# JuliaGaussianProcesses/AbstractGPs.jl

Measured on NVIDIA H100. Metric: ms to logpdf(fx,y)+posterior(fx,y), lower is better.
Workload: dtype f64

## Files before the change

abstractgps.jl_b200/csrc/engine.cu:

```cuda
#include <cuda_runtime.h>
#include <math.h>
#include <stdio.h>
#include <stdlib.h>
#include <string.h>
#include <functional>
#include <string>
#include <type_traits>
#include <utility>
#include <vector>

#include <nccl.h>

#include "agp.h"
#include "kernels.h"
#include "umma_ozaki.h"

#define TILE AGP_TILE

struct agp_ctx {
  int device = 0;
  cudaStream_t stream = nullptr;
  cudaStream_t stream2 = nullptr;
  cudaStream_t stream3 = nullptr;
  cudaEvent_t ev_s3 = nullptr, ev_fac = nullptr;
  bool s3_dirty = false;
  std::vector<cudaEvent_t> dep_ev;
  agp_config cfg{};
  std::string err;
  int64_t info = 0;
  int memspace = AGP_MEM_HOST;
  bool out_dev_override = false;
  double timings[8] = {0, 0, 0, 0, 0, 0, 0, 0};
  cudaEvent_t ev[8]{};
  std::vector<cudaEvent_t> prof_ev;
  int prof_used = 0;
  int profile = 1;
  int rank = 0, nranks = 1, grid_p = 1, grid_q = 1;
  ncclComm_t nccl = nullptr;
  OzakiWs oz{};
  OzakiWs oz2{};
  int64_t oz_rows = 0, oz2_rows = 0;
  cudaStream_t stream_comm = nullptr;
  int oz_S = 6;
  int oz_chunk = 16;
  int oz_S32 = 4;
};

struct CompState {
  CompositeDesc desc{};
  std::vector<double> w;
  int64_t grad_len = 5;
  bool owns_w = false;
};

struct agp_post {
  agp_ctx* ctx = nullptr;
  int dtype = AGP_F64;
  int64_t n = 0, n_pad = 0, lda = 0;
  int D = 0;
  void* L = nullptr;
  void* Dinv = nullptr;
  void* Xt = nullptr;
  void* alpha = nullptr;
  void* ard = nullptr;
  void* delta = nullptr;
  unsigned char* valid = nullptr;
  std::vector<std::pair<int64_t, int64_t>> segs;
  agp_kernel k{};
  int mean_kind = 0;
  double mean_c = 0.0;
  double logdet = 0.0;
  int dist_R = 0, dist_me = 0, dist_G = 0, dist_nloc = 0;
  int64_t dist_W = 0;
  void* Lloc = nullptr;
  void* Dinv_loc = nullptr;
  CompState* comp = nullptr;
};

struct agp_vfe_post {
  agp_ctx* ctx = nullptr;
  int dtype = AGP_F32;
  int64_t m = 0, m_pad = 0, lda = 0;
  int D = 0;
  void* U = nullptr;
  void* Udinv = nullptr;
  void* Lam = nullptr;
  void* Ldinv = nullptr;
  void* Zt = nullptr;
  void* m_e = nullptr;
  void* ard = nullptr;
  agp_kernel k{};
  int mean_kind = 0;
  double mean_c = 0.0;
};

namespace {

static inline int64_t round_up(int64_t x, int64_t m) { return (x + m - 1) / m * m; }
static inline int64_t env_int64(const char* name, int64_t dflt) {
  const char* v = getenv(name);
  return v ? atoll(v) : dflt;
}

#define CK(call)                                                                          \
  do {                                                                                    \
    cudaError_t _e = (call);                                                              \
    if (_e != cudaSuccess) {                                                              \
      char _b[512];                                                                       \
      snprintf(_b, sizeof(_b), "%s:%d %s -> %s", __FILE__, __LINE__, #call, cudaGetErrorString(_e)); \
      ctx->err = _b;                                                                      \
      return AGP_ERR_CUDA;                                                                \
    }                                                                                     \
  } while (0)

#define CKN(call)                                                                         \
  do {                                                                                    \
    ncclResult_t _r = (call);                                                             \
    if (_r != ncclSuccess) {                                                              \
      char _b[512];                                                                       \
      snprintf(_b, sizeof(_b), "%s:%d %s -> %s", __FILE__, __LINE__, #call, ncclGetErrorString(_r)); \
      ctx->err = _b;                                                                      \
      return AGP_ERR_NCCL;                                                                \
    }                                                                                     \
  } while (0)

template <typename T> struct NcclType;
template <> struct NcclType<float> { static constexpr ncclDataType_t v = ncclFloat; };
template <> struct NcclType<double> { static constexpr ncclDataType_t v = ncclDouble; };

struct Scratch {
  agp_ctx* ctx;
  std::vector<void*> ptrs;
  explicit Scratch(agp_ctx* c) : ctx(c) {}
  ~Scratch() { for (void* p : ptrs) cudaFreeAsync(p, ctx->stream); }
  cudaError_t alloc(void** p, size_t bytes) {
    if (bytes == 0) bytes = 16;
    cudaError_t e = cudaMallocAsync(p, bytes, ctx->stream);
    if (e == cudaSuccess) ptrs.push_back(*p);
    return e;
  }
  void release(void* p) {
    for (auto& q : ptrs) if (q == p) { q = ptrs.back(); ptrs.pop_back(); return; }
  }
};

template <typename T>
int upload(agp_ctx* ctx, Scratch& sc, const void* src, size_t count, bool always_host, T** out) {
  if (!src || count == 0) { *out = nullptr; return AGP_OK; }
  if (!always_host && ctx->memspace == AGP_MEM_DEVICE) { *out = (T*)src; return AGP_OK; }
  void* d = nullptr;
  CK(sc.alloc(&d, count * sizeof(T)));
  CK(cudaMemcpyAsync(d, src, count * sizeof(T), cudaMemcpyHostToDevice, ctx->stream));
  *out = (T*)d;
  return AGP_OK;
}

template <typename T>
int download(agp_ctx* ctx, void* dst, const T* src, size_t count, bool always_host) {
  if (!dst || count == 0) return AGP_OK;
  cudaMemcpyKind kind = (!always_host && (ctx->memspace == AGP_MEM_DEVICE || ctx->out_dev_override)) ? cudaMemcpyDeviceToDevice : cudaMemcpyDeviceToHost;
  CK(cudaMemcpyAsync(dst, src, count * sizeof(T), kind, ctx->stream));
  return AGP_OK;
}

int check_kernel(agp_ctx* ctx, const agp_kernel* k, int D) {
  if (!k) { ctx->err = "kernel spec is NULL"; return AGP_ERR_INVALID; }
  if (k->family == AGP_COMPOSITE) {
    if (ctx->nccl) { ctx->err = "composite kernels are supported on a single-GPU context only"; return AGP_ERR_UNSUPPORTED; }
    if (k->transform != AGP_T_NONE || k->variance != 1.0) {
      ctx->err = "a composite kernel takes transform AGP_T_NONE and variance 1 (scalings belong to the terms)";
      return AGP_ERR_INVALID;
    }
    if (D <= 0) { ctx->err = "D must be positive"; return AGP_ERR_DIM_MISMATCH; }
    return AGP_OK;
  }
  if (k->family < AGP_SE || k->family > AGP_LINEAR) { ctx->err = "unsupported kernel family"; return AGP_ERR_UNSUPPORTED; }
  if (k->transform < AGP_T_NONE || k->transform > AGP_T_ARD) { ctx->err = "unsupported transform"; return AGP_ERR_UNSUPPORTED; }
  if (k->transform == AGP_T_ARD && !k->ard) { ctx->err = "ARD transform without weights"; return AGP_ERR_INVALID; }
  if (D <= 0) { ctx->err = "D must be positive"; return AGP_ERR_DIM_MISMATCH; }
  return AGP_OK;
}

template <typename T>
int comp_build(agp_ctx* ctx, const agp_kernel* k, int D, CompState* cs) {
  const agp_kernel_composite* c = k->composite;
  if (!c || !c->nfactors || !c->variance || !c->factors) { ctx->err = "composite kernel without its descriptor"; return AGP_ERR_INVALID; }
  if (k->transform != AGP_T_NONE || k->variance != 1.0) {
    ctx->err = "a composite kernel takes transform AGP_T_NONE and variance 1 (scalings belong to the terms)";
    return AGP_ERR_INVALID;
  }
  if (c->nterms < 1 || c->nterms > AGP_COMP_MAX) { ctx->err = "composite kernel: 1..8 terms"; return AGP_ERR_INVALID; }
  int nf = 0;
  for (int t = 0; t < c->nterms; ++t) {
    if (c->nfactors[t] < 1) { ctx->err = "composite kernel: every term needs at least one factor"; return AGP_ERR_INVALID; }
    nf += c->nfactors[t];
    if (nf > AGP_COMP_MAX) { ctx->err = "composite kernel: at most 8 factors in all"; return AGP_ERR_INVALID; }
  }
  CompositeDesc& d = cs->desc;
  d = CompositeDesc{};
  d.nterms = c->nterms;
  d.nfactors = nf;
  cs->w.clear();
  int raw_sq = -1, raw_dot = -1;
  auto new_acc = [&](int kind) {
    const int a = d.nacc++;
    d.acc_kind[a] = kind;
    cs->w.resize((size_t)2 * d.nacc * D, 0.0);
    for (int i = 0; i < D; ++i) cs->w[(size_t)2 * a * D + i] = 1.0;
    return a;
  };
  int64_t slot = 5;
  int f = 0;
  for (int t = 0; t < c->nterms; ++t) {
    d.variance[t] = c->variance[t];
    d.g_var[t] = (int)slot++;
    for (int j = 0; j < c->nfactors[t]; ++j, ++f) {
      const agp_kernel_factor& in = c->factors[f];
      CompFactor& F = d.f[f];
      F.family = in.family; F.transform = in.transform; F.term = t;
      F.s = in.transform == AGP_T_SCALE ? in.scale : 1.0;
      F.s2 = 1.0; F.param = in.param;
      F.g_s = F.g_p = F.g_w = F.g_r = -1;
      if (in.family < AGP_SE || in.family > AGP_CONSTANT) { ctx->err = "composite kernel: unsupported factor family"; return AGP_ERR_UNSUPPORTED; }
      if (in.transform < AGP_T_NONE || in.transform > AGP_T_ARD) { ctx->err = "composite kernel: unsupported factor transform"; return AGP_ERR_UNSUPPORTED; }
      if (in.transform == AGP_T_ARD && !in.ard) { ctx->err = "composite kernel: ARD factor without weights"; return AGP_ERR_INVALID; }
      if (in.family == AGP_RQ && !(in.param > 0.0)) { ctx->err = "composite kernel: RationalQuadratic alpha must be > 0"; return AGP_ERR_INVALID; }
      const T* ard = (const T*)in.ard;
      if (in.family == AGP_CONSTANT) {
        F.acc = -1;
      } else if (in.family == AGP_PERIODIC) {
        F.acc = new_acc(COMP_ACC_PER);
        for (int i = 0; i < D; ++i) {
          const double r = in.r ? (double)((const T*)in.r)[i] : 1.0;
          if (!(r > 0.0)) { ctx->err = "composite kernel: Periodic r must be > 0"; return AGP_ERR_INVALID; }
          cs->w[(size_t)2 * F.acc * D + i] = in.transform == AGP_T_ARD ? (double)ard[i] : F.s;
          cs->w[(size_t)(2 * F.acc + 1) * D + i] = 1.0 / r;
        }
      } else if (in.transform == AGP_T_ARD) {
        F.acc = new_acc(in.family == AGP_LINEAR ? COMP_ACC_DOT : COMP_ACC_SQ);
        for (int i = 0; i < D; ++i) cs->w[(size_t)2 * F.acc * D + i] = (double)ard[i];
      } else if (in.family == AGP_LINEAR) {
        if (raw_dot < 0) raw_dot = new_acc(COMP_ACC_DOT);
        F.acc = raw_dot;
        F.s2 = F.s * F.s;
      } else {
        if (raw_sq < 0) raw_sq = new_acc(COMP_ACC_SQ);
        F.acc = raw_sq;
        F.s2 = F.s * F.s;
      }
      if (in.transform == AGP_T_SCALE) F.g_s = (int)slot++;
      else if (in.transform == AGP_T_ARD) { F.g_w = (int)slot; slot += D; }
      if (in.family == AGP_RQ || in.family == AGP_LINEAR || in.family == AGP_CONSTANT) F.g_p = (int)slot++;
      if (in.family == AGP_PERIODIC) { F.g_r = (int)slot; slot += D; }
    }
  }
  if (d.nacc == 0) new_acc(COMP_ACC_SQ);
  cs->grad_len = slot;
  return AGP_OK;
}

template <typename T>
int comp_upload(agp_ctx* ctx, Scratch& sc, CompState* cs, bool own) {
  std::vector<T> h(cs->w.begin(), cs->w.end());
  void* dv = nullptr;
  const size_t bytes = h.size() * sizeof(T);
  if (own) CK(cudaMallocAsync(&dv, bytes, ctx->stream));
  else CK(sc.alloc(&dv, bytes));
  CK(cudaMemcpyAsync(dv, h.data(), bytes, cudaMemcpyHostToDevice, ctx->stream));
  CK(cudaStreamSynchronize(ctx->stream));
  cs->desc.w = dv;
  cs->owns_w = own;
  return AGP_OK;
}

void comp_free(CompState* cs, cudaStream_t s) {
  if (!cs) return;
  if (cs->owns_w && cs->desc.w) cudaFreeAsync((void*)cs->desc.w, s);
  delete cs;
}

void prof_begin(agp_ctx* ctx) { ctx->prof_used = 0; }
cudaEvent_t prof_event(agp_ctx* ctx) {
  if (ctx->prof_used == (int)ctx->prof_ev.size()) {
    cudaEvent_t e;
    cudaEventCreate(&e);
    ctx->prof_ev.push_back(e);
  }
  return ctx->prof_ev[ctx->prof_used++];
}
double prof_total_ms(agp_ctx* ctx) {
  double t = 0;
  for (int i = 0; i + 1 < ctx->prof_used; i += 2) {
    float ms = 0;
    if (cudaEventElapsedTime(&ms, ctx->prof_ev[i], ctx->prof_ev[i + 1]) == cudaSuccess) t += ms;
  }
  return t;
}

static cudaEvent_t dep_event(agp_ctx* ctx, size_t i) {
  while (ctx->dep_ev.size() <= i) {
    cudaEvent_t e;
    cudaEventCreateWithFlags(&e, cudaEventDisableTiming);
    ctx->dep_ev.push_back(e);
  }
  return ctx->dep_ev[i];
}

template <typename T>
void trailing_update(agp_ctx* ctx, T* L, int64_t lda, int64_t row0, int64_t col0, int64_t kcol0, int64_t K,
                     int64_t M, int64_t N, cudaStream_t st, const OzakiWs* oz = nullptr, int64_t oz_row0 = 0) {
  if (M <= 0 || N <= 0) return;
  if (ctx->profile) cudaEventRecord(prof_event(ctx), st);
  bool done = false;
  if (oz) {
    if constexpr (std::is_same<T, double>::value) {
      done = ozaki_syrk(*oz, L + row0 + col0 * lda, lda, M, N, 1, 0, 0, col0 - oz_row0, row0 - oz_row0, st) == 0;
    } else {
      done = ozaki_update_ex(*oz, L + row0 + col0 * lda, 1, lda, M, N, 0, -1.0, 0, 0, col0 - oz_row0, row0 - oz_row0, st) == 0;
    }
  }
  if (!done) {
    GemmArgs u{};
    u.A = L + row0 + kcol0 * lda; u.lda = lda;
    u.B = L + row0 + kcol0 * lda; u.ldb = lda;
    u.C = L + row0 + col0 * lda; u.ldc = lda;
    u.M = M; u.N = N; u.K = K; u.alpha_neg = 1; u.beta_one = 1; u.lower_only = 1;
    if (row0 != col0) { u.b_tile_stride = TILE; u.b_off = col0 - row0; }
    launch_gemm<T>(u, st);
  }
  if (ctx->profile) cudaEventRecord(prof_event(ctx), st);
}

static void join_inverses(agp_ctx* ctx) {
  if (!ctx->s3_dirty) return;
  cudaEventRecord(ctx->ev_s3, ctx->stream3);
  cudaStreamWaitEvent(ctx->stream, ctx->ev_s3, 0);
  ctx->s3_dirty = false;
}

static int resolve_G(const agp_ctx* ctx, int64_t n_pad) {
  int nb = ctx->cfg.tile_nb;
  if (nb <= 0) nb = (n_pad >= 8192) ? 512 : TILE;
  int G = nb / TILE;
  if (G > 8) G = 8;
  return G < 1 ? 1 : G;
}
static int resolve_fp64_mode(const agp_ctx* ctx, int64_t n_pad) {
  if (ctx->cfg.fp64_mode >= 0) return ctx->cfg.fp64_mode;
  return n_pad >= 8192 ? 1 : 0;
}
static int resolve_fp32_mode(const agp_ctx* ctx, int64_t n_pad) {
  if (ctx->cfg.fp32_mode >= 0) return ctx->cfg.fp32_mode;
  return n_pad >= 4096 ? 1 : 0;
}
template <typename T> static int resolve_tensor_mode(const agp_ctx* ctx, int64_t n_pad) {
  return std::is_same<T, double>::value ? resolve_fp64_mode(ctx, n_pad) : resolve_fp32_mode(ctx, n_pad);
}
struct OzFmt { int S, bits; };
template <typename T> static OzFmt slice_format(const agp_ctx* ctx, int64_t K, bool factor) {
  if (!std::is_same<T, double>::value) return {ctx->oz_S32, 7};
  if (ctx->oz_S == 6) return (factor && K <= OZ8_MAX_K) ? OzFmt{6, 8} : OzFmt{7, 7};
  return {ctx->oz_S, 7};
}
static bool ensure_ws(OzakiWs& ws, int64_t& ws_rows, int64_t rows, int K, OzFmt f, cudaStream_t s) {
  if (!ws.SL || ws.K != K || ws_rows < rows || ws.S != f.S || ws.bits != f.bits) {
    if (ws.SL) ozaki_ws_destroy(&ws, s);
    if (ozaki_ws_create(&ws, rows, K, f.S, s, f.bits) == 0) ws_rows = rows;
    else { memset(&ws, 0, sizeof(ws)); ws_rows = 0; }
  }
  return ws.SL != nullptr;
}
template <typename T> static bool ensure_oz2(agp_ctx* ctx, int64_t rows, int K, bool factor, cudaStream_t s) {
  return ensure_ws(ctx->oz2, ctx->oz2_rows, rows, K, slice_format<T>(ctx, K, factor), s);
}
template <typename T> static bool ensure_oz(agp_ctx* ctx, int64_t rows, int K, bool factor, cudaStream_t s) {
  return ensure_ws(ctx->oz, ctx->oz_rows, rows, K, slice_format<T>(ctx, K, factor), s);
}

template <typename T>
int panel_route(int64_t rows_below) {
  if (!std::is_same<T, double>::value || !potrf_split_enabled()) return AGP_PANEL_FUSED;
  static const int64_t trsm_gemm_min = env_int64("AGP_TRSM_GEMM_MIN", 8192);
  return rows_below >= trsm_gemm_min ? AGP_PANEL_SPLIT_GEMM : AGP_PANEL_SPLIT_SUBST;
}

template <typename T>
void panel_block(agp_ctx* ctx, int route, T* Akk, int64_t lda, int64_t rows_below, T* Dinv_k, double* logdet_part,
                 int blk, int* info, cudaStream_t s) {
  if constexpr (std::is_same<T, double>::value) {
    if (route == AGP_PANEL_SPLIT_SUBST) {
      launch_potrf_factor_f64(Akk, lda, logdet_part, blk, info, s);
      cudaEventRecord(ctx->ev_fac, s);
      cudaStreamWaitEvent(ctx->stream3, ctx->ev_fac, 0);
      launch_trtri_f64(Akk, lda, Dinv_k, ctx->stream3);
      ctx->s3_dirty = true;
      if (rows_below > 0) launch_trsm_sub_f64(Akk + TILE, lda, rows_below, Akk, s);
      return;
    }
    if (route == AGP_PANEL_SPLIT_GEMM) {
      launch_potrf_factor_f64(Akk, lda, logdet_part, blk, info, s);
      launch_trtri_f64(Akk, lda, Dinv_k, s);
    }
  }
  if (route == AGP_PANEL_FUSED) launch_potrf_diag<T>(Akk, lda, Dinv_k, logdet_part, blk, info, s);
  if (rows_below > 0) {
    GemmArgs t{};
    t.A = Akk + TILE; t.lda = lda; t.B = Dinv_k; t.ldb = TILE;
    t.C = Akk + TILE; t.ldc = lda; t.M = rows_below; t.N = TILE; t.K = TILE;
    launch_gemm<T>(t, s);
  }
}

template <typename T>
void factor_panel_step(agp_ctx* ctx, T* Lp, int64_t lda, int Gp, int g, int64_t rows, T* Dinv_p, double* logdet_part,
                       int blk_base, int* info, cudaStream_t s) {
  T* Akk = Lp + (int64_t)g * TILE + (int64_t)g * TILE * lda;
  const int64_t rows_below = rows - (int64_t)(g + 1) * TILE;
  panel_block<T>(ctx, panel_route<T>(rows_below), Akk, lda, rows_below, Dinv_p + (int64_t)g * TILE * TILE, logdet_part,
                 blk_base + g, info, s);
  if (rows_below <= 0) return;
  const int64_t ncols_in = (int64_t)(Gp - (g + 1)) * TILE;
  if (ncols_in > 0) {
    GemmArgs u{};
    u.A = Akk + TILE; u.lda = lda; u.B = Akk + TILE; u.ldb = lda;
    u.C = Akk + TILE + (int64_t)TILE * lda; u.ldc = lda;
    u.M = rows_below; u.N = ncols_in; u.K = TILE; u.alpha_neg = 1; u.beta_one = 1; u.lower_only = 1;
    launch_gemm<T>(u, s);
  }
}

template <typename T>
void factor_panel(agp_ctx* ctx, T* Lp, int64_t lda, int Gp, int64_t rows, T* Dinv_p, double* logdet_part, int blk_base,
                  int* info, cudaStream_t s) {
  for (int g = 0; g < Gp; ++g) factor_panel_step<T>(ctx, Lp, lda, Gp, g, rows, Dinv_p, logdet_part, blk_base, info, s);
}

template <typename T>
void cholesky_inplace(agp_ctx* ctx, T* L, int64_t lda, int64_t n_pad, int64_t rows_total, T* Dinv,
                      double* logdet_part, int* info) {
  cudaStream_t s = ctx->stream, s2 = ctx->stream2;
  const int nblk = (int)(n_pad / TILE);
  const int fp64_mode = resolve_tensor_mode<T>(ctx, n_pad);
  int G = resolve_G(ctx, n_pad);
  if (!std::is_same<T, double>::value && fp64_mode == 1 && ctx->cfg.tile_nb <= 0 && n_pad >= 4096) G = 4;
  const bool oz_ok = fp64_mode == 1 && nblk > 2 * G && ensure_oz<T>(ctx, rows_total, G * TILE, true, s) &&
                     (std::is_same<T, double>::value || ctx->oz.bulk == 2);
  const bool la = ctx->cfg.lookahead != 0 && nblk > 2 * G;
  const bool la2 = la && ctx->cfg.lookahead >= 2;
  bool rest_pending = false, restA_pending = false, last_rest_full = false;
  size_t ev_idx = 0, last_rest = 0, last_restA = 0;
  for (int ko = 0; ko < nblk; ko += G) {
    const int g_end = (ko + G < nblk) ? ko + G : nblk;
    factor_panel<T>(ctx, L + (int64_t)ko * TILE + (int64_t)ko * TILE * lda, lda, g_end - ko, rows_total - (int64_t)ko * TILE,
                    Dinv + (int64_t)ko * TILE * TILE, logdet_part, ko, info, s);
    const int64_t t0 = (int64_t)g_end * TILE;
    const int64_t cols_trail = n_pad - t0;
    if (cols_trail <= 0) continue;
    const int64_t K = (int64_t)(g_end - ko) * TILE, kc0 = (int64_t)ko * TILE;
    const OzakiWs* oz = nullptr;
    if (oz_ok && K == ctx->oz.K && cols_trail >= 2 * TILE) oz = &ctx->oz;
    constexpr int is_f32 = std::is_same<T, double>::value ? 0 : 1;
    if (!la) {
      if (oz) ozaki_prepare_ex(*oz, L + t0 + kc0 * lda, is_f32, 0, lda, rows_total - t0, 0, s);
      trailing_update<T>(ctx, L, lda, t0, t0, kc0, K, rows_total - t0, cols_trail, s, oz, t0);
      continue;
    }
    if (la2 && !oz) {
      cudaEvent_t e_panel = dep_event(ctx, ev_idx++), e_restA = dep_event(ctx, ev_idx++), e_restB = dep_event(ctx, ev_idx++);
      if (restA_pending) cudaStreamWaitEvent(s, dep_event(ctx, last_restA), 0);
      if (rest_pending && last_rest_full) cudaStreamWaitEvent(s, dep_event(ctx, last_rest), 0);
      cudaEventRecord(e_panel, s);
      const int64_t next_cols = (cols_trail < (int64_t)G * TILE) ? cols_trail : (int64_t)G * TILE;
      trailing_update<T>(ctx, L, lda, t0, t0, kc0, K, rows_total - t0, next_cols, s, nullptr, t0);
      restA_pending = false;
      rest_pending = false;
      if (cols_trail > next_cols) {
        const int64_t r0 = t0 + next_cols;
        const int64_t colsA = (n_pad - r0 < (int64_t)G * TILE) ? (n_pad - r0) : (int64_t)G * TILE;
        cudaStreamWaitEvent(s2, e_panel, 0);
        trailing_update<T>(ctx, L, lda, r0, r0, kc0, K, rows_total - r0, colsA, s2, nullptr, t0);
        cudaEventRecord(e_restA, s2);
        restA_pending = true;
        last_restA = ev_idx - 2;
        const int64_t r1 = r0 + colsA;
        if (n_pad > r1) trailing_update<T>(ctx, L, lda, r1, r1, kc0, K, rows_total - r1, n_pad - r1, s2, nullptr, t0);
        cudaEventRecord(e_restB, s2);
        rest_pending = true;
        last_rest_full = false;
        last_rest = ev_idx - 1;
      }
      continue;
    }
    cudaEvent_t e_panel = dep_event(ctx, ev_idx++), e_rest = dep_event(ctx, ev_idx++);
    if (rest_pending) cudaStreamWaitEvent(s, dep_event(ctx, last_rest), 0);
    if (restA_pending) { cudaStreamWaitEvent(s, dep_event(ctx, last_restA), 0); restA_pending = false; }
    if (oz) ozaki_prepare_ex(*oz, L + t0 + kc0 * lda, is_f32, 0, lda, rows_total - t0, 0, s);
    cudaEventRecord(e_panel, s);
    const int64_t next_cols = (cols_trail < (int64_t)G * TILE) ? cols_trail : (int64_t)G * TILE;
    trailing_update<T>(ctx, L, lda, t0, t0, kc0, K, rows_total - t0, next_cols, s, oz, t0);
    rest_pending = false;
    if (cols_trail > next_cols) {
      const int64_t r0 = t0 + next_cols;
      cudaStreamWaitEvent(s2, e_panel, 0);
      if (oz) oz->chunk_tiles = ctx->oz_chunk;
      trailing_update<T>(ctx, L, lda, r0, r0, kc0, K, rows_total - r0, n_pad - r0, s2, oz, t0);
      if (oz) oz->chunk_tiles = 0;
      cudaEventRecord(e_rest, s2);
      rest_pending = true;
      last_rest_full = true;
      last_rest = ev_idx - 1;
    }
  }
  if (rest_pending) cudaStreamWaitEvent(s, dep_event(ctx, last_rest), 0);
  join_inverses(ctx);
}

template <typename T>
bool forward_subst_multi_tc(agp_ctx* ctx, const T* L, int64_t lda, const T* Dinv, int64_t n_pad, T* B, int64_t ldb,
                            int64_t ncols) {
  cudaStream_t s = ctx->stream;
  constexpr int GW = 4;
  const int64_t W = (int64_t)GW * TILE;
  const int nblk = (int)(n_pad / TILE);
  constexpr int is_f32 = std::is_same<T, double>::value ? 0 : 1;
  const int64_t a_rows = round_up(n_pad, TILE);
  if (!ensure_oz<T>(ctx, a_rows + ncols, (int)W, false, s) || ctx->oz.bulk != 2) return false;
  const OzakiWs& ws = ctx->oz;
  for (int ko = 0; ko < nblk; ko += GW) {
    const int k_end = (ko + GW < nblk) ? ko + GW : nblk;
    const int64_t blk_end = (int64_t)k_end * TILE;
    for (int k = ko; k < k_end; ++k) {
      T* Bk = B + (int64_t)k * TILE;
      GemmArgs a{};
      a.A = Dinv + (int64_t)k * TILE * TILE; a.lda = TILE; a.a_kmajor = 0;
      a.B = Bk; a.ldb = ldb; a.b_kmajor = 1;
      a.C = Bk; a.ldc = ldb; a.M = TILE; a.N = ncols; a.K = TILE;
      launch_gemm<T>(a, s);
      const int64_t rows_in = blk_end - (int64_t)(k + 1) * TILE;
      if (rows_in <= 0) continue;
      GemmArgs u{};
      u.A = L + (int64_t)(k + 1) * TILE + (int64_t)k * TILE * lda; u.lda = lda; u.a_kmajor = 0;
      u.B = Bk; u.ldb = ldb; u.b_kmajor = 1;
      u.C = Bk + TILE; u.ldc = ldb; u.M = rows_in; u.N = ncols; u.K = TILE; u.alpha_neg = 1; u.beta_one = 1;
      launch_gemm<T>(u, s);
    }
    const int64_t rows_below = n_pad - blk_end, Kw = blk_end - (int64_t)ko * TILE;
    if (rows_below <= 0) continue;
    if (Kw != W) {
      GemmArgs u{};
      u.A = L + blk_end + (int64_t)ko * TILE * lda; u.lda = lda; u.a_kmajor = 0;
      u.B = B + (int64_t)ko * TILE; u.ldb = ldb; u.b_kmajor = 1;
      u.C = B + blk_end; u.ldc = ldb; u.M = rows_below; u.N = ncols; u.K = Kw; u.alpha_neg = 1; u.beta_one = 1;
      launch_gemm<T>(u, s);
      continue;
    }
    ozaki_prepare_ex(ws, L + blk_end + (int64_t)ko * TILE * lda, is_f32, 0, lda, rows_below, 0, s);
    ozaki_prepare_ex(ws, B + (int64_t)ko * TILE, is_f32, 1, ldb, ncols, a_rows, s);
    if (ozaki_update_ex(ws, B + blk_end, is_f32, ldb, rows_below, ncols, 1, -1.0, 0, 0, a_rows, 0, s) != 0) return false;
  }
  return true;
}

template <typename T>
void forward_subst_multi(agp_ctx* ctx, const T* L, int64_t lda, const T* Dinv, int64_t n_pad, T* B, int64_t ldb,
                         int64_t ncols) {
  cudaStream_t s = ctx->stream;
  const int nblk = (int)(n_pad / TILE);
  static const int64_t tc_min_cols = env_int64("AGP_SOLVE_TC_MIN_COLS", 512);
  if (resolve_tensor_mode<T>(ctx, n_pad >= 2048 ? (int64_t)1 << 20 : 0) == 1 && n_pad >= 2048 && ncols % TILE == 0 &&
      ncols >= tc_min_cols) {
    if (forward_subst_multi_tc<T>(ctx, L, lda, Dinv, n_pad, B, ldb, ncols)) return;
  }
  for (int k = 0; k < nblk; ++k) {
    T* Bk = B + (int64_t)k * TILE;
    GemmArgs a{};
    a.A = Dinv + (int64_t)k * TILE * TILE; a.lda = TILE; a.a_kmajor = 0;
    a.B = Bk; a.ldb = ldb; a.b_kmajor = 1;
    a.C = Bk; a.ldc = ldb; a.M = TILE; a.N = ncols; a.K = TILE;
    launch_gemm<T>(a, s);
    const int64_t rows_below = n_pad - (int64_t)(k + 1) * TILE;
    if (rows_below <= 0) continue;
    GemmArgs u{};
    u.A = L + (int64_t)(k + 1) * TILE + (int64_t)k * TILE * lda; u.lda = lda; u.a_kmajor = 0;
    u.B = Bk; u.ldb = ldb; u.b_kmajor = 1;
    u.C = Bk + TILE; u.ldc = ldb; u.M = rows_below; u.N = ncols; u.K = TILE; u.alpha_neg = 1; u.beta_one = 1;
    launch_gemm<T>(u, s);
  }
}

template <typename T>
bool backward_subst_multi_tc(agp_ctx* ctx, const T* L, int64_t lda, const T* Dinv, int64_t n_pad, T* B, int64_t ldb,
                             int64_t ncols) {
  cudaStream_t s = ctx->stream;
  constexpr int GW = 4;
  const int64_t W = (int64_t)GW * TILE;
  const int nblk = (int)(n_pad / TILE);
  constexpr int is_f32 = std::is_same<T, double>::value ? 0 : 1;
  const int64_t a_rows = round_up(n_pad, TILE);
  if (!ensure_oz<T>(ctx, a_rows + ncols, (int)W, false, s) || ctx->oz.bulk != 2) return false;
  const OzakiWs& ws = ctx->oz;
  for (int ko = (nblk - 1) / GW * GW; ko >= 0; ko -= GW) {
    const int k_end = (ko + GW < nblk) ? ko + GW : nblk;
    const int64_t blk0 = (int64_t)ko * TILE;
    for (int k = k_end - 1; k >= ko; --k) {
      T* Bk = B + (int64_t)k * TILE;
      GemmArgs a{};
      a.A = Dinv + (int64_t)k * TILE * TILE; a.lda = TILE; a.a_kmajor = 1;
      a.B = Bk; a.ldb = ldb; a.b_kmajor = 1;
      a.C = Bk; a.ldc = ldb; a.M = TILE; a.N = ncols; a.K = TILE;
      launch_gemm<T>(a, s);
      const int64_t rows_in = (int64_t)k * TILE - blk0;
      if (rows_in <= 0) continue;
      GemmArgs u{};
      u.A = L + (int64_t)k * TILE + blk0 * lda; u.lda = lda; u.a_kmajor = 1;
      u.B = Bk; u.ldb = ldb; u.b_kmajor = 1;
      u.C = B + blk0; u.ldc = ldb; u.M = rows_in; u.N = ncols; u.K = TILE; u.alpha_neg = 1; u.beta_one = 1;
      launch_gemm<T>(u, s);
    }
    const int64_t rows_above = blk0, Kw = (int64_t)k_end * TILE - blk0;
    if (rows_above <= 0) continue;
    if (Kw != W) {
      GemmArgs u{};
      u.A = L + blk0; u.lda = lda; u.a_kmajor = 1;
      u.B = B + blk0; u.ldb = ldb; u.b_kmajor = 1;
      u.C = B; u.ldc = ldb; u.M = rows_above; u.N = ncols; u.K = Kw; u.alpha_neg = 1; u.beta_one = 1;
      launch_gemm<T>(u, s);
      continue;
    }
    ozaki_prepare_ex(ws, L + blk0, is_f32, 1, lda, rows_above, 0, s);
    ozaki_prepare_ex(ws, B + blk0, is_f32, 1, ldb, ncols, a_rows, s);
    if (ozaki_update_ex(ws, B, is_f32, ldb, rows_above, ncols, 1, -1.0, 0, 0, a_rows, 0, s) != 0) return false;
  }
  return true;
}

template <typename T>
void backward_subst_multi(agp_ctx* ctx, const T* L, int64_t lda, const T* Dinv, int64_t n_pad, T* B, int64_t ldb,
                          int64_t ncols) {
  cudaStream_t s = ctx->stream;
  const int nblk = (int)(n_pad / TILE);
  static const int64_t tc_min_cols = env_int64("AGP_SOLVE_TC_MIN_COLS", 512);
  if (resolve_tensor_mode<T>(ctx, n_pad >= 2048 ? (int64_t)1 << 20 : 0) == 1 && n_pad >= 2048 && ncols % TILE == 0 &&
      ncols >= tc_min_cols) {
    if (backward_subst_multi_tc<T>(ctx, L, lda, Dinv, n_pad, B, ldb, ncols)) return;
  }
  for (int k = nblk - 1; k >= 0; --k) {
    T* Bk = B + (int64_t)k * TILE;
    GemmArgs a{};
    a.A = Dinv + (int64_t)k * TILE * TILE; a.lda = TILE; a.a_kmajor = 1;
    a.B = Bk; a.ldb = ldb; a.b_kmajor = 1;
    a.C = Bk; a.ldc = ldb; a.M = TILE; a.N = ncols; a.K = TILE;
    launch_gemm<T>(a, s);
    const int64_t rows_above = (int64_t)k * TILE;
    if (rows_above <= 0) continue;
    GemmArgs u{};
    u.A = L + (int64_t)k * TILE; u.lda = lda; u.a_kmajor = 1;
    u.B = Bk; u.ldb = ldb; u.b_kmajor = 1;
// ... 2500 lines not shown
      if (oz && (int64_t)(nto - 1 - kk) * W >= 2 * TILE) {
        ozaki_prepare(*oz, (const double*)Pk, rows_below, rows_below, s);
        use_oz = true;
      }
    }
    cudaEvent_t e_panel = dep_event(ctx, ev_idx++), e_rest = dep_event(ctx, ev_idx++);
    cudaEventRecord(e_panel, s);
    const int lj_first = local_first_after(kk);
    int lj_bulk = lj_first;
    if ((kk + 1) % R == me) {
      trailing(kk, Pk, lj_first, lj_first + 1, use_oz, s);
      lj_bulk = lj_first + 1;
    }
    rest_pending = true;
    last_rest = ev_idx - 1;
    if (sched2 && (kk + 1) % R == me) {
      def = DeferredRest{true, kk, Pk, lj_bulk, nloc, use_oz, e_rest};
    } else {
      cudaStreamWaitEvent(s2, e_panel, 0);
      rest_update(kk, Pk, lj_bulk, nloc, use_oz, e_rest);
    }
  }
  if (rest_pending) cudaStreamWaitEvent(s, dep_event(ctx, last_rest), 0);
  join_inverses(ctx);
  CK(cudaEventRecord(ctx->ev[3], s));

  for (int lj = 0; lj < nloc; ++lj) {
    const int64_t jo = (int64_t)lj * R + me;
    for (int sI = 0; sI < S; ++sI)
      launch_copy2d<T>(L + n_pad + sI + (int64_t)lj * W * lda, lda, rwork + (size_t)sI * n_pad + jo * W, 1, 1, W, s);
  }
  for (int sI = 0; sI < S; ++sI) launch_sumsq<T>(rwork + (size_t)sI * n_pad, n_pad, dscal + nt + sI, s);
  if (R > 1) CKN(ncclAllReduce(dscal, dscal, (size_t)(nt + TILE), ncclDouble, ncclSum, ctx->nccl, s));
  {
    int pending = -1;
    for (int io = nto - 1; io >= 0; --io) {
      const int owner = io % R, i_lo = io * G;
      const int64_t p_lo = (int64_t)(pending >= 0 ? pending : 0) * G;
      T* a_pend = alpha + p_lo * TILE;
      if (owner == me) {
        if (pending >= 0)
          launch_bwd_update_local_multi<T>(L, lda, (int)p_lo, G, a_pend, rwork, nloc * G, me, R, G, i_lo, (int64_t)i_lo + G, s);
        launch_bwd_block_solve<T>(L + (int64_t)io * W + (int64_t)(io / R) * W * lda, lda, Dinv + (int64_t)(io / R) * G * TILE * TILE,
                                  rwork + (int64_t)i_lo * TILE, alpha + (int64_t)i_lo * TILE, G, s);
      } else if (pending >= 0) {
        launch_bwd_update_local_multi<T>(L, lda, (int)p_lo, G, a_pend, rwork, nloc * G, me, R, G, 0, p_lo, s);
      }
      if (R > 1) CKN(ncclAllReduce(alpha + (int64_t)i_lo * TILE, alpha + (int64_t)i_lo * TILE, (size_t)G * TILE, NcclType<T>::v, ncclSum, ctx->nccl, s));
      if (owner == me && pending >= 0)
        launch_bwd_update_local_multi<T>(L, lda, (int)p_lo, G, a_pend, rwork, nloc * G, me, R, G, 0, i_lo, s);
      pending = io;
    }
  }
  launch_finalize_logpdf<T>(dscal, nt, dscal + nt, S, N, lp_d, dscal + nt + TILE, s);
  CK(cudaEventRecord(ctx->ev[4], s));
  int h_info = 0;
  if (R > 1) CKN(ncclAllReduce(dinfo, dinfo, 1, ncclInt, ncclMax, ctx->nccl, s));
  CK(cudaMemcpyAsync(&h_info, dinfo, sizeof(int), cudaMemcpyDeviceToHost, s));
  if (logpdf_out) CK(cudaMemcpyAsync(logpdf_out, lp_d, (size_t)S * sizeof(T), cudaMemcpyDeviceToHost, s));
  if (alpha_out) { rc = download<T>(ctx, alpha_out, alpha, (size_t)N, false); if (rc) return rc; }
  CK(cudaEventRecord(ctx->ev[5], s));
  CK(cudaStreamSynchronize(s));
  CK(cudaStreamSynchronize(s2));
  CK(cudaGetLastError());
  float ms = 0;
  auto el = [&](int a, int b) { cudaEventElapsedTime(&ms, ctx->ev[a], ctx->ev[b]); return (double)ms; };
  ctx->timings[0] = el(0, 5); ctx->timings[1] = el(0, 1); ctx->timings[2] = el(1, 2); ctx->timings[3] = el(2, 3);
  ctx->timings[4] = el(3, 4); ctx->timings[5] = el(4, 5); ctx->timings[6] = 0.0;
  ctx->timings[7] = ctx->profile ? prof_total_ms(ctx) : 0.0;
  if (h_info != 0) {
    ctx->info = h_info;
    ctx->err = "matrix is not positive definite (distributed Cholesky)";
    return AGP_ERR_NOT_POSDEF;
  }
  if (keep) {
    CK(cudaMallocAsync(&post->alpha, (size_t)n_pad * sizeof(T), s));
    CK(cudaMallocAsync(&post->delta, (size_t)n_pad * sizeof(T), s));
    CK(cudaMemcpyAsync(post->alpha, alpha, (size_t)n_pad * sizeof(T), cudaMemcpyDeviceToDevice, s));
    CK(cudaMemsetAsync(post->delta, 0, (size_t)n_pad * sizeof(T), s));
    launch_sub_mean<T>(Yd, N, mean->kind, mean->c, mean_d, (T*)post->delta, s);
    double h_logdet = 0.0;
    CK(cudaMemcpyAsync(&h_logdet, dscal + nt + TILE, sizeof(double), cudaMemcpyDeviceToHost, s));
    CK(cudaStreamSynchronize(s));
    post->logdet = h_logdet;
    guard.p = nullptr;
    *post_out = post;
  }
  return AGP_OK;
}

int env_int(const char* name, int dflt) {
  const char* v = getenv(name);
  return v ? atoi(v) : dflt;
}

}

#define DISPATCH(dtype, call_f32, call_f64)                                   \
  ((dtype) == AGP_F32 ? (call_f32) : ((dtype) == AGP_F64 ? (call_f64) : (int)AGP_ERR_UNSUPPORTED))

extern "C" {

const char* agp_version(void) { return "agp-blackwell 0.1 (sm_90a)"; }

int32_t agp_init(agp_ctx** out, int32_t device, const agp_config* cfg) {
  if (!out) return AGP_ERR_INVALID;
  *out = nullptr;
  int ndev = 0;
  if (cudaGetDeviceCount(&ndev) != cudaSuccess || ndev == 0) return AGP_ERR_CUDA;
  if (device < 0 || device >= ndev) return AGP_ERR_INVALID;
  agp_ctx* ctx = new agp_ctx();
  ctx->device = device;
  if (cfg) ctx->cfg = *cfg;
  ctx->cfg.tile_nb = env_int("AGP_NB", (cfg && cfg->tile_nb > 0) ? cfg->tile_nb : 0);
  if (ctx->cfg.tile_nb % TILE) ctx->cfg.tile_nb = 0;
  ctx->cfg.fp64_mode = env_int("AGP_FP64_MODE", cfg ? ctx->cfg.fp64_mode : -1);
  ctx->cfg.fp32_mode = env_int("AGP_FP32_MODE", cfg ? ctx->cfg.fp32_mode : -1);
  ctx->cfg.lookahead = env_int("AGP_LOOKAHEAD", cfg ? ctx->cfg.lookahead : 2);
  ctx->cfg.use_graph = env_int("AGP_GRAPH", ctx->cfg.use_graph);
  ctx->profile = env_int("AGP_PROFILE", cfg ? cfg->profile_kernels : 0);
  ctx->oz_S = env_int("AGP_OZAKI_S", (cfg && cfg->ozaki_slices) ? cfg->ozaki_slices : 6);
  if (ctx->oz_S < 5 || ctx->oz_S > 8) ctx->oz_S = 6;
  ctx->oz_S32 = env_int("AGP_OZAKI_S32", 4);
  if (ctx->oz_S32 < 3 || ctx->oz_S32 > 5) ctx->oz_S32 = 4;
  if (cudaSetDevice(device) != cudaSuccess) { delete ctx; return AGP_ERR_CUDA; }
  int prio_lo = 0, prio_hi = 0;
  cudaDeviceGetStreamPriorityRange(&prio_lo, &prio_hi);
  if (cudaStreamCreateWithPriority(&ctx->stream, cudaStreamNonBlocking, prio_hi) != cudaSuccess) { delete ctx; return AGP_ERR_CUDA; }
  if (cudaStreamCreateWithPriority(&ctx->stream2, cudaStreamNonBlocking, prio_lo) != cudaSuccess) { delete ctx; return AGP_ERR_CUDA; }
  if (cudaStreamCreateWithPriority(&ctx->stream3, cudaStreamNonBlocking, prio_hi) != cudaSuccess) { delete ctx; return AGP_ERR_CUDA; }
  ctx->oz_chunk = env_int("AGP_OZAKI_CHUNK", 16);
  if (ctx->oz_chunk < 0 || ctx->oz_chunk > 4096) ctx->oz_chunk = 16;
  cudaEventCreateWithFlags(&ctx->ev_s3, cudaEventDisableTiming);
  cudaEventCreateWithFlags(&ctx->ev_fac, cudaEventDisableTiming);
  for (int i = 0; i < 8; ++i) cudaEventCreate(&ctx->ev[i]);
  cudaMemPool_t pool;
  if (cudaDeviceGetDefaultMemPool(&pool, device) == cudaSuccess) {
    uint64_t thr = UINT64_MAX;
    cudaMemPoolSetAttribute(pool, cudaMemPoolAttrReleaseThreshold, &thr);
  }
  *out = ctx;
  return AGP_OK;
}

int32_t agp_destroy(agp_ctx* ctx) {
  if (!ctx) return AGP_OK;
  cudaSetDevice(ctx->device);
  cudaStreamSynchronize(ctx->stream);
  for (int i = 0; i < 8; ++i) cudaEventDestroy(ctx->ev[i]);
  for (auto e : ctx->prof_ev) cudaEventDestroy(e);
  for (auto e : ctx->dep_ev) cudaEventDestroy(e);
  if (ctx->oz.SL) ozaki_ws_destroy(&ctx->oz, ctx->stream);
  if (ctx->oz2.SL) ozaki_ws_destroy(&ctx->oz2, ctx->stream);
  if (ctx->stream_comm) { cudaStreamSynchronize(ctx->stream_comm); cudaStreamDestroy(ctx->stream_comm); }
  if (ctx->nccl) ncclCommDestroy(ctx->nccl);
  cudaEventDestroy(ctx->ev_s3);
  cudaEventDestroy(ctx->ev_fac);
  cudaStreamDestroy(ctx->stream3);
  cudaStreamDestroy(ctx->stream2);
  cudaStreamDestroy(ctx->stream);
  delete ctx;
  return AGP_OK;
}

const char* agp_last_error(const agp_ctx* ctx) { return ctx ? ctx->err.c_str() : "null ctx"; }
int64_t agp_last_info(const agp_ctx* ctx) { return ctx ? ctx->info : 0; }
int32_t agp_set_memspace(agp_ctx* ctx, int32_t m) {
  if (!ctx || (m != AGP_MEM_HOST && m != AGP_MEM_DEVICE)) return AGP_ERR_INVALID;
  ctx->memspace = m;
  return AGP_OK;
}
int32_t agp_set_config(agp_ctx* ctx, const agp_config* cfg) {
  if (!ctx || !cfg) return AGP_ERR_INVALID;
  if (cfg->tile_nb < 0 || cfg->tile_nb % TILE) return AGP_ERR_INVALID;
  ctx->cfg.tile_nb = cfg->tile_nb;
  ctx->cfg.fp64_mode = cfg->fp64_mode;
  ctx->cfg.fp32_mode = cfg->fp32_mode;
  ctx->cfg.lookahead = cfg->lookahead;
  ctx->profile = cfg->profile_kernels;
  if (cfg->ozaki_slices >= 5 && cfg->ozaki_slices <= 8) { ctx->cfg.ozaki_slices = cfg->ozaki_slices; ctx->oz_S = cfg->ozaki_slices; }
  return AGP_OK;
}
int32_t agp_get_config(const agp_ctx* ctx, agp_config* out) {
  if (!ctx || !out) return AGP_ERR_INVALID;
  *out = ctx->cfg;
  out->ozaki_slices = ctx->oz_S;
  out->profile_kernels = ctx->profile;
  return AGP_OK;
}
int32_t agp_last_timings(const agp_ctx* ctx, double* out, int32_t n) {
  if (!ctx || !out) return 0;
  int c = n < 8 ? n : 8;
  for (int i = 0; i < c; ++i) out[i] = ctx->timings[i];
  return c;
}
int64_t agp_launch_count(const agp_ctx*) { return agp_kernel_launches(); }

int32_t agp_gram(agp_ctx* ctx, int32_t dtype, const agp_kernel* k, int32_t layout, const void* X, int64_t N,
                 int32_t D, const void* Z, int64_t M, const agp_noise* noise, void* K_out) {
  if (!ctx) return AGP_ERR_INVALID;
  return DISPATCH(dtype, gram_impl<float>(ctx, k, layout, X, N, D, Z, M, noise, K_out),
                  gram_impl<double>(ctx, k, layout, X, N, D, Z, M, noise, K_out));
}

int32_t agp_fit(agp_ctx* ctx, int32_t dtype, const agp_kernel* k, const agp_mean* mean, const agp_noise* noise,
                int32_t layout, const void* X, int64_t N, int32_t D, const void* Y, int32_t S, void* logpdf_out,
                void* alpha_out, agp_post** post_out) {
  if (!ctx) return AGP_ERR_INVALID;
  if (post_out) *post_out = nullptr;
  if (ctx->nccl) {
    return DISPATCH(dtype, fit_dist_impl<float>(ctx, k, mean, noise, layout, X, N, D, Y, S, logpdf_out, alpha_out, post_out),
                    fit_dist_impl<double>(ctx, k, mean, noise, layout, X, N, D, Y, S, logpdf_out, alpha_out, post_out));
  }
  return DISPATCH(dtype, fit_many_impl<float>(ctx, k, mean, noise, layout, X, N, D, Y, S, logpdf_out, alpha_out, post_out),
                  fit_many_impl<double>(ctx, k, mean, noise, layout, X, N, D, Y, S, logpdf_out, alpha_out, post_out));
}

int32_t agp_post_mean_var(agp_post* p, int32_t layout, const void* Xs, int64_t M, const agp_mean* mean_s,
                          const agp_noise* noise_s, void* mean_out, void* var_out) {
  if (!p) return AGP_ERR_INVALID;
  if (p->dist_R > 1)
    return DISPATCH(p->dtype, post_mean_var_dist<float>(p, layout, Xs, M, mean_s, noise_s, mean_out, var_out),
                    post_mean_var_dist<double>(p, layout, Xs, M, mean_s, noise_s, mean_out, var_out));
  return DISPATCH(p->dtype, post_mean_var_impl<float>(p, layout, Xs, M, mean_s, noise_s, mean_out, var_out),
                  post_mean_var_impl<double>(p, layout, Xs, M, mean_s, noise_s, mean_out, var_out));
}

int32_t agp_post_mean_cov(agp_post* p, int32_t layout, const void* Xs, int64_t M, const agp_mean* mean_s,
                          void* mean_out, void* cov_out) {
  if (!p) return AGP_ERR_INVALID;
  return DISPATCH(p->dtype, post_mean_cov_impl<float>(p, layout, Xs, M, mean_s, mean_out, cov_out),
                  post_mean_cov_impl<double>(p, layout, Xs, M, mean_s, mean_out, cov_out));
}

int32_t agp_post_logpdf(agp_post* p, int32_t layout, const void* Xs, int64_t M, const agp_mean* mean_s,
                        const agp_noise* noise_s, const void* Y, int32_t S, void* logpdf_out) {
  if (!p) return AGP_ERR_INVALID;
  if (S <= 0) { p->ctx->err = "S must be positive"; return AGP_ERR_INVALID; }
  return DISPATCH(p->dtype, post_cond_impl<float>(p, layout, Xs, M, mean_s, noise_s, Y, S, logpdf_out, nullptr, 0, nullptr),
                  post_cond_impl<double>(p, layout, Xs, M, mean_s, noise_s, Y, S, logpdf_out, nullptr, 0, nullptr));
}

int32_t agp_post_rand(agp_post* p, int32_t layout, const void* Xs, int64_t M, const agp_mean* mean_s,
                      const agp_noise* noise_s, const void* Z, int32_t S, void* out) {
  if (!p) return AGP_ERR_INVALID;
  if (S <= 0) return AGP_OK;
  return DISPATCH(p->dtype, post_cond_impl<float>(p, layout, Xs, M, mean_s, noise_s, nullptr, 0, nullptr, Z, S, out),
                  post_cond_impl<double>(p, layout, Xs, M, mean_s, noise_s, nullptr, 0, nullptr, Z, S, out));
}

int32_t agp_post_logpdf_grad(agp_post* p, double* grad_out, void* noise_diag_out) {
  if (!p || !grad_out) return AGP_ERR_INVALID;
  return agp_post_logpdf_grad_x(p, grad_out, noise_diag_out, AGP_POINT_MAJOR, nullptr);
}

int32_t agp_post_logpdf_grad_x(agp_post* p, double* grad_out, void* noise_diag_out, int32_t layout, void* x_grad_out) {
  if (!p) return AGP_ERR_INVALID;
  return DISPATCH(p->dtype, post_logpdf_grad_impl<float>(p, grad_out, noise_diag_out, layout, x_grad_out),
                  post_logpdf_grad_impl<double>(p, grad_out, noise_diag_out, layout, x_grad_out));
}

int32_t agp_post_logpdf_grad_cols(agp_post* p, const agp_mean* mean, const void* Y, int32_t S, const double* lp_bar,
                                  double* grad_out, void* noise_diag_out, void* mean_diag_out, int32_t layout,
                                  void* x_grad_out, void* y_bar_out) {
  if (!p) return AGP_ERR_INVALID;
  return DISPATCH(p->dtype,
                  post_logpdf_grad_cols_impl<float>(p, mean, Y, S, lp_bar, grad_out, noise_diag_out, mean_diag_out, layout,
                                                    x_grad_out, y_bar_out),
                  post_logpdf_grad_cols_impl<double>(p, mean, Y, S, lp_bar, grad_out, noise_diag_out, mean_diag_out, layout,
                                                     x_grad_out, y_bar_out));
}

int32_t agp_post_pred_logpdf_grad(agp_post* p, int32_t layout, const void* Xs, int64_t M, const agp_mean* mean_s,
                                  const agp_noise* noise_s, const void* Ys, int32_t S, const double* lp_bar, void* lp_out,
                                  double* grad_out, void* noise_diag_out, void* mean_diag_out, void* y_bar_out,
                                  void* x_grad_out, void* noise_s_diag_out, void* mean_s_diag_out, void* ys_bar_out,
                                  void* xs_grad_out) {
  if (!p) return AGP_ERR_INVALID;
  return DISPATCH(p->dtype,
                  post_pred_logpdf_grad_impl<float>(p, layout, Xs, M, mean_s, noise_s, Ys, S, lp_bar, lp_out, grad_out,
                                                    noise_diag_out, mean_diag_out, y_bar_out, x_grad_out, noise_s_diag_out,
                                                    mean_s_diag_out, ys_bar_out, xs_grad_out),
                  post_pred_logpdf_grad_impl<double>(p, layout, Xs, M, mean_s, noise_s, Ys, S, lp_bar, lp_out, grad_out,
                                                     noise_diag_out, mean_diag_out, y_bar_out, x_grad_out, noise_s_diag_out,
                                                     mean_s_diag_out, ys_bar_out, xs_grad_out));
}

int32_t agp_post_rand_grad(agp_post* p, int32_t layout, const void* Xs, int64_t M, const agp_mean* mean_s,
                           const agp_noise* noise_s, const void* Z, int32_t S, const void* out_bar, double* grad_out,
                           void* noise_diag_out, void* mean_diag_out, void* y_bar_out, void* x_grad_out,
                           void* noise_s_diag_out, void* mean_s_diag_out, void* z_bar_out, void* xs_grad_out) {
  if (!p) return AGP_ERR_INVALID;
  return DISPATCH(p->dtype,
                  post_rand_grad_impl<float>(p, layout, Xs, M, mean_s, noise_s, Z, S, out_bar, grad_out, noise_diag_out,
                                             mean_diag_out, y_bar_out, x_grad_out, noise_s_diag_out, mean_s_diag_out,
                                             z_bar_out, xs_grad_out),
                  post_rand_grad_impl<double>(p, layout, Xs, M, mean_s, noise_s, Z, S, out_bar, grad_out, noise_diag_out,
                                              mean_diag_out, y_bar_out, x_grad_out, noise_s_diag_out, mean_s_diag_out,
                                              z_bar_out, xs_grad_out));
}

int32_t agp_post_mean_var_grad(agp_post* p, int32_t layout, const void* Xs, int64_t M, const void* mean_bar,
                               const void* var_bar, double* grad_out, void* noise_diag_out, void* mean_diag_out,
                               void* y_bar_out, void* x_grad_out, void* xs_grad_out) {
  if (!p) return AGP_ERR_INVALID;
  return DISPATCH(p->dtype,
// ... 333 lines not shown
```

Measured before the change: 1939.

## Use 1024-wide outer panels with Ozaki-accelerated split panel factorization for large f64

For large f64 problems (n_pad of at least 32768) using the 6-slice Ozaki mode, the outer block size rises from 512 to 1024 columns. Each wide outer panel is factored as two halves, with the inner update between them done by a second Ozaki workspace using 8-bit slices. The lookahead chunk size for the trailing update on the second stream is scaled down in proportion to K. The intent is fewer outer iterations and larger, more efficient trailing GEMMs, at the cost of a longer serial panel and an extra workspace allocation.

```diff
diff --git a/abstractgps.jl_b200/csrc/engine.cu b/abstractgps.jl_b200/csrc/engine.cu
--- a/abstractgps.jl_b200/csrc/engine.cu
+++ b/abstractgps.jl_b200/csrc/engine.cu
@@ -39,7 +39,8 @@
   ncclComm_t nccl = nullptr;
   OzakiWs oz{};
   OzakiWs oz2{};
-  int64_t oz_rows = 0, oz2_rows = 0;
+  OzakiWs ozp{};
+  int64_t oz_rows = 0, oz2_rows = 0, ozp_rows = 0;
   cudaStream_t stream_comm = nullptr;
   int oz_S = 6;
   int oz_chunk = 16;
@@ -345,6 +346,7 @@
   if (G > 8) G = 8;
   return G < 1 ? 1 : G;
 }
+constexpr int64_t AUTO_NB1024_MIN = 32768;
 static int resolve_fp64_mode(const agp_ctx* ctx, int64_t n_pad) {
   if (ctx->cfg.fp64_mode >= 0) return ctx->cfg.fp64_mode;
   return n_pad >= 8192 ? 1 : 0;
@@ -436,6 +438,23 @@
 }
 
 template <typename T>
+void factor_outer_panel(agp_ctx* ctx, T* L, int64_t lda, int ko, int Gp, int64_t rows_total, T* Dinv,
+                        double* logdet_part, int* info, cudaStream_t s, const OzakiWs* ozp) {
+  const int64_t p0 = (int64_t)ko * TILE;
+  if (!ozp || (int64_t)Gp * TILE != 2 * (int64_t)ozp->K) {
+    factor_panel<T>(ctx, L + p0 + p0 * lda, lda, Gp, rows_total - p0, Dinv + p0 * TILE, logdet_part, ko, info, s);
+    return;
+  }
+  const int h = Gp / 2;
+  const int64_t h0 = p0 + (int64_t)h * TILE;
+  factor_panel<T>(ctx, L + p0 + p0 * lda, lda, h, rows_total - p0, Dinv + p0 * TILE, logdet_part, ko, info, s);
+  constexpr int is_f32 = std::is_same<T, double>::value ? 0 : 1;
+  ozaki_prepare_ex(*ozp, L + h0 + p0 * lda, is_f32, 0, lda, rows_total - h0, 0, s);
+  trailing_update<T>(ctx, L, lda, h0, h0, p0, ozp->K, rows_total - h0, (int64_t)(Gp - h) * TILE, s, ozp, h0);
+  factor_panel<T>(ctx, L + h0 + h0 * lda, lda, Gp - h, rows_total - h0, Dinv + h0 * TILE, logdet_part, ko + h, info, s);
+}
+
+template <typename T>
 void cholesky_inplace(agp_ctx* ctx, T* L, int64_t lda, int64_t n_pad, int64_t rows_total, T* Dinv,
                       double* logdet_part, int* info) {
   cudaStream_t s = ctx->stream, s2 = ctx->stream2;
@@ -443,16 +462,23 @@
   const int fp64_mode = resolve_tensor_mode<T>(ctx, n_pad);
   int G = resolve_G(ctx, n_pad);
   if (!std::is_same<T, double>::value && fp64_mode == 1 && ctx->cfg.tile_nb <= 0 && n_pad >= 4096) G = 4;
+  if (std::is_same<T, double>::value && fp64_mode == 1 && ctx->cfg.tile_nb <= 0 && ctx->oz_S == 6 &&
+      n_pad >= AUTO_NB1024_MIN)
+    G = 8;
   const bool oz_ok = fp64_mode == 1 && nblk > 2 * G && ensure_oz<T>(ctx, rows_total, G * TILE, true, s) &&
                      (std::is_same<T, double>::value || ctx->oz.bulk == 2);
+  const OzakiWs* ozp = nullptr;
+  if (oz_ok && ctx->oz.bits == 8 && G > 4 && G % 2 == 0 &&
+      ensure_ws(ctx->ozp, ctx->ozp_rows, rows_total, G / 2 * TILE, slice_format<T>(ctx, G / 2 * TILE, true), s) &&
+      ctx->ozp.bits == 8)
+    ozp = &ctx->ozp;
   const bool la = ctx->cfg.lookahead != 0 && nblk > 2 * G;
   const bool la2 = la && ctx->cfg.lookahead >= 2;
   bool rest_pending = false, restA_pending = false, last_rest_full = false;
   size_t ev_idx = 0, last_rest = 0, last_restA = 0;
   for (int ko = 0; ko < nblk; ko += G) {
     const int g_end = (ko + G < nblk) ? ko + G : nblk;
-    factor_panel<T>(ctx, L + (int64_t)ko * TILE + (int64_t)ko * TILE * lda, lda, g_end - ko, rows_total - (int64_t)ko * TILE,
-                    Dinv + (int64_t)ko * TILE * TILE, logdet_part, ko, info, s);
+    factor_outer_panel<T>(ctx, L, lda, ko, g_end - ko, rows_total, Dinv, logdet_part, info, s, ozp);
     const int64_t t0 = (int64_t)g_end * TILE;
     const int64_t cols_trail = n_pad - t0;
     if (cols_trail <= 0) continue;
@@ -502,7 +528,7 @@
     if (cols_trail > next_cols) {
       const int64_t r0 = t0 + next_cols;
       cudaStreamWaitEvent(s2, e_panel, 0);
-      if (oz) oz->chunk_tiles = ctx->oz_chunk;
+      if (oz) oz->chunk_tiles = K > 512 && ctx->oz_chunk > 0 ? std::max(1, (int)(ctx->oz_chunk * 512 / K)) : ctx->oz_chunk;
       trailing_update<T>(ctx, L, lda, r0, r0, kc0, K, rows_total - r0, n_pad - r0, s2, oz, t0);
       if (oz) oz->chunk_tiles = 0;
       cudaEventRecord(e_rest, s2);
@@ -3309,6 +3335,7 @@
   for (auto e : ctx->dep_ev) cudaEventDestroy(e);
   if (ctx->oz.SL) ozaki_ws_destroy(&ctx->oz, ctx->stream);
   if (ctx->oz2.SL) ozaki_ws_destroy(&ctx->oz2, ctx->stream);
+  if (ctx->ozp.SL) ozaki_ws_destroy(&ctx->ozp, ctx->stream);
   if (ctx->stream_comm) { cudaStreamSynchronize(ctx->stream_comm); cudaStreamDestroy(ctx->stream_comm); }
   if (ctx->nccl) ncclCommDestroy(ctx->nccl);
   cudaEventDestroy(ctx->ev_s3);
```

Result: faster. 1700 (median of 6 runs) (-12.4%).
